# aymenboudhina/Multimodal_VQVAE_compression_audio_tactile

Hardware: AMD Instinct MI355X
Metric: encode+VQ+decode token-frames/sec (1 frame = 13.33 ms of paired 24 kHz audio+tactile) (higher is better)
Workload: dtype f32

## Files before the change

include/mvq.h:

```cpp
#ifndef MVQ_H
#define MVQ_H

#include <stddef.h>
#include <stdint.h>

#ifdef __cplusplus
extern "C" {
#endif

#define MVQ_OK 0
#define MVQ_EINVAL (-1)
#define MVQ_EUNSUPPORTED (-2)
#define MVQ_EHIP (-3)

#define MVQ_ACT_NONE 0
#define MVQ_ACT_TANH 1
#define MVQ_ACT_GELU 2

int mvq_abi_version(void);
const char* mvq_last_error(void);
unsigned mvq_build_flags(void);

typedef struct mvq_profile_entry {
    char kernel[96];
    double seconds;
    double flops;
    int launches;
} mvq_profile_entry;
int mvq_profile_begin(void);
int mvq_profile_end(mvq_profile_entry* out, int max_entries, int* n_entries);
int mvq_profile_end2(mvq_profile_entry* out, int max_entries, int* n_entries, int* n_total);
int mvq_profile_reserve(int n_launches);
int mvq_device_query(int* cu_count, int* lds_bytes_per_cu, char* arch, int arch_len);


int mvq_weight_norm_f32(const float* v, const float* g, float* w, int rows, int inner, void* stream);

size_t mvq_conv1d_packed_floats(int cin, int cout, int ks);
int mvq_conv1d_pack_f32(const float* w, float* wp, int cin, int cout, int ks, void* stream);

size_t mvq_conv_transpose1d_packed_floats(int cin, int cout, int stride);
int mvq_conv_transpose1d_pack_f32(const float* w, float* wp, int cin, int cout, int stride, void* stream);


int mvq_conv1d_f32(const float* x, const float* wp, const float* bias, const float* alpha_in,
                   const float* residual, const float* alpha_out, float* y,
                   int batch, int cin, int tin, int cout, int ks, int stride, int dil, int pad, int act,
                   void* stream);

int mvq_conv1d_dual_f32(const float* x, const float* wp, const float* bias, const float* alpha_in,
                        const float* residual, const float* alpha_out, float* y, float* y2, const float* alpha2,
                        int batch, int cin, int tin, int cout, int ks, int stride, int dil, int pad, int act,
                        void* stream);
int mvq_conv_transpose1d_dual_f32(const float* x, const float* wp, const float* bias, const float* alpha_in,
                                  const float* alpha_out, float* y, float* y2, const float* alpha2,
                                  int batch, int cin, int tin, int cout, int stride, int pad, void* stream);

int mvq_conv_kernel_name(int batch, int cin, int cout, int ks, int stride, int dil, int transposed, int tin,
                         char* buf, int len);

size_t mvq_residual_unit_scratch_floats(int batch, int c, int t, int dil);
int mvq_residual_unit_kernel_name(int c, int dil, char* buf, int len);
int mvq_residual_unit_f32(const float* x, const float* w7p, const float* b7, const float* alpha_a,
                          const float* alpha_b, const float* w1p, const float* b1, const float* alpha_next,
                          float* y, float* scratch, int batch, int c, int t, int dil, void* stream);

int mvq_residual_unit_dual_f32(const float* x, const float* x_snaked, const float* w7p, const float* b7,
                               const float* alpha_a, const float* alpha_b, const float* w1p, const float* b1,
                               const float* alpha_next, float* y, float* y2, const float* alpha2, float* scratch,
                               int batch, int c, int t, int dil, void* stream);

int mvq_conv_transpose1d_f32(const float* x, const float* wp, const float* bias, const float* alpha_in,
                             const float* alpha_out, float* y,
                             int batch, int cin, int tin, int cout, int stride, int pad, void* stream);


int mvq_rvq_ema_forward_f32(const float* z, const float* books, float* q_out, int32_t* idx_out,
                            int batch, int dim, int t, int nb_use, int k, void* stream);

size_t mvq_rvq_ema_step_scratch_bytes(int batch, int t, int nb, int k, int dim);
int mvq_rvq_ema_step_f32(const float* z_tokens, float* books, void* scratch,
                         int batch, int dim, int t, int nb, int k, float decay, void* stream);

int mvq_dac_rvq_f32(const float* z, const float* in_w, const float* in_b, const float* codebook,
                    const float* out_w, const float* out_b, float* zq, int32_t* codes, float* latents,
                    int batch, int c, int t, int nq_use, int k, int dc, void* stream);
int mvq_dac_rvq_items_f32(const float* z, const float* in_w, const float* in_b, const float* codebook,
                          const float* out_w, const float* out_b, float* zq, int32_t* codes, float* latents,
                          const int32_t* nq_item, int batch, int c, int t, int nq_use, int k, int dc, void* stream);
int mvq_dac_rvq_prepare_f32(const float* codebook, float* cb_normalised, float* cb_norm2, int nq, int k, int dc, void* stream);
int mvq_dac_rvq_prepared_f32(const float* z, const float* in_w, const float* in_b, const float* codebook,
                             const float* cb_normalised, const float* cb_norm2,
                             const float* out_w, const float* out_b, float* zq, int32_t* codes, float* latents,
                             const int32_t* nq_item, int batch, int c, int t, int nq_use, int k, int dc, void* stream);


int mvq_rvq_dequant_f32(const int64_t* idx, const float* books, float* q_out, int batch, int dim, int t, int nb_use, int k,
                        size_t out_sb, size_t out_sd, void* stream);
int mvq_dac_rvq_from_codes_f32(const int64_t* codes, const float* codebook, const float* out_w, const float* out_b, float* zq,
                               float* z_p, int batch, int c, int t, int nq_use, int k, int dc, void* stream);

int mvq_idx_pack_packets_u8(const int64_t* idx, uint8_t* bodies, int batch, int nb, int t, int k, int packet_tok,
                            size_t s_book, size_t s_item, void* stream);
int mvq_idx_unpack_packets(const uint8_t* bodies, const uint8_t* nb_recv, int64_t* idx, uint8_t* nb_valid, int batch, int nb, int t,
                           int k, int packet_tok, void* stream);
int mvq_rvq_dequant_layers_f32(const int64_t* idx, const float* books, const uint8_t* nb_valid, float* q_out, int batch, int dim,
                               int t, int nb_use, int k, size_t out_sb, size_t out_sd, void* stream);

#define MVQ_RATE_FULL 0
#define MVQ_RATE_TOL2 1
#define MVQ_RATE_BUDGET 2
int mvq_rvq_rate_f32(const float* z, size_t z_sb, size_t z_sd, const int32_t* idx, size_t idx_sbook, size_t idx_sitem,
// ... 257 lines not shown
```

multimodal_vqvae_compression_audio_tactile_amd/_lib.py:

```python
from __future__ import annotations

import ctypes
import subprocess
from ctypes import c_char_p, c_float, c_int, c_size_t, c_void_p
from pathlib import Path

_PKG = Path(__file__).resolve().parent
import os as _os
SO_PATH = Path(_os.environ["MVQ_LIB_PATH"]).resolve() if _os.environ.get("MVQ_LIB_PATH") else _PKG / "libmvq_hip.so"
_lib = None

class EncoderDesc(ctypes.Structure):
    _fields_ = [("d_model", c_int), ("n_strides", c_int), ("strides", c_int * 8), ("d_latent", c_int)]


class DecoderDesc(ctypes.Structure):
    _fields_ = [("input_channel", c_int), ("channels", c_int), ("n_rates", c_int), ("rates", c_int * 8), ("d_out", c_int), ("output_padding", c_int)]


class ArArgs(ctypes.Structure):
    _fields_ = ([(n, c_int) for n in ("batch", "t_lat", "t_audio", "tactile_only", "books_use", "rvq_k", "c_lat", "c_ff", "code_dim", "heads", "chunk")]
                + [(n, c_float) for n in ("ln_eps", "tok_eps", "scale")]
                + [(n, c_void_p) for n in ("zt", "k_all", "v_all", "pe", "lnq_g", "lnq_b", "wq", "wo", "lnf_g", "lnf_b", "w1", "b1", "w3", "b3",
                                           "tok_g", "tok_b", "wd", "bd", "wu", "bu", "books", "z_run", "r_tokens", "idx_out")])


class ProfileEntry(ctypes.Structure):
    _fields_ = [("kernel", ctypes.c_char * 96), ("seconds", ctypes.c_double), ("flops", ctypes.c_double), ("launches", c_int)]


EXPORTS = {
    "mvq_profile_begin": (c_int, []),
    "mvq_profile_end": (c_int, [ctypes.POINTER(ProfileEntry), c_int, ctypes.POINTER(c_int)]),
    "mvq_profile_end2": (c_int, [ctypes.POINTER(ProfileEntry), c_int, ctypes.POINTER(c_int), ctypes.POINTER(c_int)]),
    "mvq_profile_reserve": (c_int, [c_int]),
    "mvq_abi_version": (c_int, []),
    "mvq_build_flags": (ctypes.c_uint, []),
    "mvq_last_error": (c_char_p, []),
    "mvq_device_query": (c_int, [ctypes.POINTER(c_int), ctypes.POINTER(c_int), c_char_p, c_int]),
    "mvq_weight_norm_f32": (c_int, [c_void_p, c_void_p, c_void_p, c_int, c_int, c_void_p]),
    "mvq_conv1d_packed_floats": (c_size_t, [c_int, c_int, c_int]),
    "mvq_conv1d_pack_f32": (c_int, [c_void_p, c_void_p, c_int, c_int, c_int, c_void_p]),
    "mvq_conv_transpose1d_packed_floats": (c_size_t, [c_int, c_int, c_int]),
    "mvq_conv_transpose1d_pack_f32": (c_int, [c_void_p, c_void_p, c_int, c_int, c_int, c_void_p]),
    "mvq_conv_kernel_name": (c_int, [c_int] * 8 + [c_char_p, c_int]),
    "mvq_conv1d_f32": (c_int, [c_void_p] * 7 + [c_int] * 9 + [c_void_p]),
    "mvq_bf16x3_split_bytes": (c_size_t, [c_int] * 3),
    "mvq_bf16x3_split_f32": (c_int, [c_void_p, c_void_p, c_int, c_int, c_int, c_void_p]),
    "mvq_conv1d_k7_bf16x3_packed_bytes": (c_size_t, [c_int] * 2),
    "mvq_conv1d_k7_pack_bf16x3": (c_int, [c_void_p, c_void_p, c_int, c_int, c_int, c_void_p]),
    "mvq_conv1d_k7_bf16x6_f32": (c_int, [c_void_p] * 9 + [c_int] * 6 + [c_void_p]),
    "mvq_f16x2_split_f32": (c_int, [c_void_p, c_void_p, c_void_p, c_int, c_int, c_int, c_void_p]),
    "mvq_conv1d_k7_f16x2_packed_bytes": (c_size_t, [c_int] * 2),
    "mvq_conv1d_k7_pack_f16x2": (c_int, [c_void_p, c_void_p, c_void_p, c_int, c_int, c_int, c_void_p]),
    "mvq_conv1d_k7_f16x3_f32": (c_int, [c_void_p] * 11 + [c_int] * 6 + [c_void_p]),
    "mvq_residual_unit_scratch_floats": (c_size_t, [c_int] * 4),
    "mvq_residual_unit_kernel_name": (c_int, [c_int, c_int, c_char_p, c_int]),
    "mvq_residual_unit_f32": (c_int, [c_void_p] * 10 + [c_int] * 4 + [c_void_p]),
    "mvq_conv1d_dual_f32": (c_int, [c_void_p] * 9 + [c_int] * 9 + [c_void_p]),
    "mvq_conv_transpose1d_dual_f32": (c_int, [c_void_p] * 8 + [c_int] * 6 + [c_void_p]),
    "mvq_residual_unit_dual_f32": (c_int, [c_void_p] * 13 + [c_int] * 4 + [c_void_p]),
    "mvq_conv_transpose1d_f32": (c_int, [c_void_p] * 6 + [c_int] * 6 + [c_void_p]),
    "mvq_rvq_ema_forward_f32": (c_int, [c_void_p] * 4 + [c_int] * 5 + [c_void_p]),
    "mvq_rvq_ema_step_scratch_bytes": (c_size_t, [c_int] * 5),
    "mvq_rvq_ema_step_f32": (c_int, [c_void_p] * 3 + [c_int] * 5 + [c_float, c_void_p]),
    "mvq_dac_rvq_f32": (c_int, [c_void_p] * 9 + [c_int] * 6 + [c_void_p]),
    "mvq_dac_rvq_items_f32": (c_int, [c_void_p] * 10 + [c_int] * 6 + [c_void_p]),
    "mvq_dac_rvq_prepare_f32": (c_int, [c_void_p] * 3 + [c_int] * 3 + [c_void_p]),
    "mvq_dac_rvq_prepared_f32": (c_int, [c_void_p] * 12 + [c_int] * 6 + [c_void_p]),
    "mvq_rvq_dequant_f32": (c_int, [c_void_p] * 3 + [c_int] * 5 + [c_size_t] * 2 + [c_void_p]),
    "mvq_dac_rvq_from_codes_f32": (c_int, [c_void_p] * 6 + [c_int] * 6 + [c_void_p]),
    "mvq_idx_pack_packets_u8": (c_int, [c_void_p] * 2 + [c_int] * 5 + [c_size_t] * 2 + [c_void_p]),
    "mvq_idx_unpack_packets": (c_int, [c_void_p] * 4 + [c_int] * 5 + [c_void_p]),
    "mvq_fec_parity_u8": (c_int, [c_void_p] * 3 + [c_int] * 7 + [c_void_p]),
    "mvq_fec_recover_u8": (c_int, [c_void_p] * 5 + [c_int] * 7 + [c_void_p]),
    "mvq_fec_rs_parity_u8": (c_int, [c_void_p] * 3 + [c_int] * 8 + [c_void_p]),
    "mvq_fec_rs_recover_u8": (c_int, [c_void_p] * 5 + [c_int] * 8 + [c_void_p]),
    "mvq_rvq_dequant_layers_f32": (c_int, [c_void_p] * 4 + [c_int] * 5 + [c_size_t] * 2 + [c_void_p]),
    "mvq_rvq_rate_f32": (c_int, [c_void_p, c_size_t, c_size_t, c_void_p, c_size_t, c_size_t, c_void_p, c_void_p, c_size_t, c_size_t, c_void_p,
                                 c_size_t, c_void_p, c_size_t, c_void_p] + [c_int] * 9 + [c_float, c_int, c_void_p]),
    "mvq_dac_rvq_from_codes_layers_f32": (c_int, [c_void_p, c_size_t] + [c_void_p] * 6 + [c_int] * 6 + [c_void_p]),
    "mvq_dac_rvq_rate_workspace_bytes": (c_size_t, [c_int] * 4),
    "mvq_dac_rvq_rate_f32": (c_int, [c_void_p, c_void_p, c_size_t] + [c_void_p] * 8 + [c_size_t] + [c_int] * 9 + [c_float, c_int, c_void_p]),
    "mvq_layernorm_c_f32": (c_int, [c_void_p] * 5 + [c_int] * 3 + [c_size_t] * 2 + [c_float, c_int, c_float, c_void_p]),
    "mvq_attention_f32": (c_int, [c_void_p] * 4 + [c_int] * 5 + [c_size_t] * 4 + [c_void_p]),
    "mvq_align_xcorr_f32": (c_int, [c_void_p, c_void_p, c_int, c_int, c_void_p, c_void_p, c_void_p, c_void_p]),
    "mvq_align_xcorr_batch_f32": (c_int, [c_void_p, c_void_p, c_int, c_int, c_int, c_void_p, c_void_p, c_void_p, c_void_p]),
    "mvq_resample_ragged_f32": (c_int, [c_void_p] * 6 + [c_int] * 7 + [c_void_p]),
    "mvq_conv1d_dgrad_packed_floats": (c_size_t, [c_int] * 3),
    "mvq_conv1d_pack_dgrad_f32": (c_int, [c_void_p, c_void_p, c_int, c_int, c_int, c_void_p]),
    "mvq_conv_transpose1d_pack_dgrad_f32": (c_int, [c_void_p, c_void_p, c_int, c_int, c_int, c_void_p]),
    "mvq_conv1d_dgrad_f32": (c_int, [c_void_p] * 6 + [c_int] * 9 + [c_void_p]),
    "mvq_mul_dtanh_f32": (c_int, [c_void_p, c_void_p, c_void_p, c_size_t, c_void_p]),
    "mvq_layernorm_c_bwd_f32": (c_int, [c_void_p] * 8 + [c_int] * 3 + [c_size_t] * 2 + [c_float, c_void_p]),
    "mvq_gelu_bwd_f32": (c_int, [c_void_p, c_void_p, c_void_p, c_size_t, c_void_p]),
    "mvq_scale_tanh_f32": (c_int, [c_void_p, c_float, c_void_p, c_size_t, c_void_p]),
    "mvq_scale_tanh_bwd_f32": (c_int, [c_void_p, c_void_p, c_float, c_void_p, c_void_p, c_int, c_size_t, c_void_p]),
    "mvq_attention_bwd_f32": (c_int, [c_void_p] * 7 + [c_int] * 5 + [c_size_t] * 4 + [c_void_p]),
# ... 130 lines not shown
```

multimodal_vqvae_compression_audio_tactile_amd/csrc/api.hip:

```cpp
#include <hip/hip_runtime.h>
#include <stdarg.h>
#include <math.h>
#include <stdio.h>
#include <string.h>
#include "../../include/mvq.h"
#include "conv_dispatch.hpp"
#include "kernels_small.hpp"

#include <map>
#include <string>
#include <vector>

namespace mvq {
namespace {
struct ProfRec { std::string name; double flops; hipEvent_t e0, e1; };
std::vector<ProfRec> g_prof;
std::vector<hipEvent_t> g_prof_pool;
bool g_prof_on = false;
hipError_t g_prof_err = hipSuccess;
hipEvent_t prof_event()
{
    if (!g_prof_pool.empty()) { hipEvent_t e = g_prof_pool.back(); g_prof_pool.pop_back(); return e; }
    hipEvent_t e = nullptr;
    const hipError_t rc = hipEventCreate(&e);
// ... 260 lines not shown
size_t mvq_conv1d_k7_f16x2_packed_bytes(int cout, int cin)
{
    if (cout <= 0 || cin <= 0 || mvq::bf16x6_tile_rows(cout) == 0 || cin % 16 != 0) return 0;
    return (size_t)cout * cin * 7 * 4;
}
int mvq_conv1d_k7_pack_f16x2(const float* w, void* wq, uint32_t* wamax, int cout, int cin, int dgrad, void* stream)
{
    if (cout <= 0 || cin <= 0 || mvq::bf16x6_tile_rows(cout) == 0 || cin % 16 != 0)
        return fail(MVQ_EINVAL, "conv1d_k7_pack_f16x2: Cout %d must be a multiple of 128 or 96 and Cin %d of 16", cout, cin);
    if (!w || !wq || !wamax) return fail(MVQ_EINVAL, "conv1d_k7_pack_f16x2: null tensor");
    if ((reinterpret_cast<uintptr_t>(wq) & 15) != 0) return fail(MVQ_EINVAL, "conv1d_k7_pack_f16x2: wq must be 16-byte aligned");
    const hipError_t e = mvq::launch_f16x2_pack_k7(w, wq, wamax, cout, cin, dgrad != 0, S(stream));
    return e == hipSuccess ? MVQ_OK : hipfail(e, "conv1d_k7_pack_f16x2");
}
int mvq_conv1d_k7_f16x3_f32(const void* xs, const uint32_t* xamax, const void* wq, const uint32_t* wamax, const float* bias,
                            const float* alpha_out, float* y, float* y2, const float* dsn_src, const float* dsn_alpha,
                            const float* residual, int batch, int cin, int t, int cout, int dil, int tvalid, void* stream)
{
    if (batch < 0 || cin <= 0 || cout <= 0 || t < 0 || mvq::bf16x6_tile_rows(cout) == 0 || cin % 16 != 0)
        return fail(MVQ_EINVAL, "conv1d_k7_f16x3: bad shape B=%d Cin=%d T=%d Cout=%d (Cout %% 128 or 96, Cin %% 16)", batch, cin, t, cout);
    if (dil != 1 && dil != 3 && dil != 9) return fail(MVQ_EINVAL, "conv1d_k7_f16x3: dilation %d not in {1, 3, 9}", dil);
    if (tvalid < 0 || tvalid > t) return fail(MVQ_EINVAL, "conv1d_k7_f16x3: tvalid %d outside [0, %d]", tvalid, t);
    if (batch == 0 || t == 0) return MVQ_OK;
    if (!xs || !wq || !y || !xamax || !wamax) return fail(MVQ_EINVAL, "conv1d_k7_f16x3: null tensor");
    if (((reinterpret_cast<uintptr_t>(xs) | reinterpret_cast<uintptr_t>(wq)) & 15) != 0)
        return fail(MVQ_EINVAL, "conv1d_k7_f16x3: xs / wq must be 16-byte aligned");
    if ((long long)batch * ((t + 127) / 128) > 0x7fffffffLL) return fail(MVQ_EINVAL, "conv1d_k7_f16x3: grid too large");
    if (y2 && !alpha_out) return fail(MVQ_EINVAL, "conv1d_k7_f16x3: the dual output needs alpha_out");
    if ((dsn_src != nullptr) != (dsn_alpha != nullptr)) return fail(MVQ_EINVAL, "conv1d_k7_f16x3: dsn_src and dsn_alpha go together");
    mvq::K7Extra ex; ex.y2 = y2; ex.dsn_src = dsn_src; ex.dsn_alpha = dsn_alpha; ex.residual = residual;
    const hipError_t e = mvq::launch_conv_k7_f16x3(xs, xamax, wq, wamax, bias, alpha_out, y, batch, cin, t, cout, dil, tvalid, ex, S(stream));
    return e == hipSuccess ? MVQ_OK : hipfail(e, "conv1d_k7_f16x3");
}

int mvq_conv_kernel_name(int batch, int cin, int cout, int ks, int stride, int dil, int transposed, int tin, char* buf, int len)
{
    if (!buf || len <= 0) return fail(MVQ_EINVAL, "conv_kernel_name: bad buffer");
    mvq::ConvArgs a{};
    a.B = batch; a.Cin = cin; a.Tin = tin; a.Cout = cout; a.name_out = buf; a.name_len = len;
    hipError_t e;
    if (transposed) {
        a.Mrows = cout * stride; a.Mpad = mvq::conv_mpad(a.Mrows); a.Ncols = tin + 1; a.up_s = stride; a.pad = 1;
        e = dispatch_convtr(a, nullptr);
        if (e != hipSuccess) snprintf(buf, len, "convtr_direct_kernel");
    } else {
        const int pad = stride == 1 ? (ks - 1) * dil / 2 : (stride + 1) / 2;
        a.Mrows = cout; a.Mpad = mvq::conv_mpad(cout); a.Ncols = conv_out_len(tin, ks, stride, dil, pad); a.pad = pad;
        a.Tout = a.Ncols; a.up_s = 1;
        e = dispatch_conv1d(a, ks, stride, dil, nullptr);
        if (e != hipSuccess)
            snprintf(buf, len, "%s", (cin == 1 && ks == 7 && stride == 1 && dil == 1) ? "conv1d_cin1_kernel<7>"
                                   : (cout == 1 && ks == 7 && stride == 1 && dil == 1) ? "conv1d_cout1_kernel<7>"
                                                                                       : "conv1d_direct_kernel");
    }
    return MVQ_OK;
}

int mvq_conv1d_dual_f32(const float* x, const float* wp, const float* bias, const float* alpha_in,
                        const float* residual, const float* alpha_out, float* y, float* y2, const float* alpha2,
                        int batch, int cin, int tin, int cout, int ks, int stride, int dil, int pad, int act, void* stream);

int mvq_conv1d_f32(const float* x, const float* wp, const float* bias, const float* alpha_in,
                   const float* residual, const float* alpha_out, float* y,
                   int batch, int cin, int tin, int cout, int ks, int stride, int dil, int pad, int act, void* stream)
{
    return mvq_conv1d_dual_f32(x, wp, bias, alpha_in, residual, alpha_out, y, nullptr, nullptr,
                               batch, cin, tin, cout, ks, stride, dil, pad, act, stream);
}

int mvq_conv1d_dual_f32(const float* x, const float* wp, const float* bias, const float* alpha_in,
                        const float* residual, const float* alpha_out, float* y, float* y2, const float* alpha2,
                        int batch, int cin, int tin, int cout, int ks, int stride, int dil, int pad, int act, void* stream)
{
    return mvq_conv1d_padded_f32(x, wp, bias, alpha_in, residual, alpha_out, y, y2, alpha2, batch, cin, tin, cout, ks, stride,
                                 dil, pad, act, 0, stream);
}

int mvq_conv1d_padded_f32(const float* x, const float* wp, const float* bias, const float* alpha_in,
                          const float* residual, const float* alpha_out, float* y, float* y2, const float* alpha2,
                          int batch, int cin, int tin, int cout, int ks, int stride, int dil, int pad, int act, int tvalid,
                          void* stream)
{
    if (batch < 0 || cin <= 0 || cout <= 0 || tin < 0 || ks <= 0 || stride <= 0 || dil <= 0 || pad < 0)
        return fail(MVQ_EINVAL, "conv1d: bad shape B=%d Cin=%d Tin=%d Cout=%d ks=%d s=%d d=%d p=%d", batch, cin, tin, cout, ks, stride, dil, pad);
    if (act != MVQ_ACT_NONE && act != MVQ_ACT_TANH && act != MVQ_ACT_GELU) return fail(MVQ_EINVAL, "conv1d: bad act %d", act);
    const int tout = conv_out_len(tin, ks, stride, dil, pad);
    if (batch == 0 || tout == 0) return MVQ_OK;
    if (!x || !wp || !y) return fail(MVQ_EINVAL, "conv1d: null tensor");
    if ((y2 != nullptr) != (alpha2 != nullptr)) return fail(MVQ_EINVAL, "conv1d: y2 and alpha2 go together");
    if (tvalid < 0 || tvalid > tout) return fail(MVQ_EINVAL, "conv1d: tvalid %d outside [0, %d]", tvalid, tout);
    const int mpad = mvq::conv_mpad(cout);

    mvq::ConvArgs a{};
    a.x = x; a.wp = wp; a.bias = bias; a.alpha_in = alpha_in; a.residual = residual; a.alpha_out = alpha_out; a.y = y;
    a.B = batch; a.Cin = cin; a.Tin = tin; a.Cout = cout; a.Tout = tout; a.pad = pad; a.Mpad = mpad;
    a.Mrows = cout; a.Ncols = tout; a.act = act; a.up_s = 1; a.up_p = 0; a.y2 = y2; a.alpha2 = alpha2;
    a.tvalid = (tvalid == tout) ? 0 : tvalid;

    hipError_t e = dispatch_conv1d(a, ks, stride, dil, S(stream));
    if (e == hipErrorInvalidValue && (a.tvalid || act == MVQ_ACT_GELU))
        return fail(MVQ_EUNSUPPORTED, "conv1d: zero-padded rows / the GELU epilogue need an MFMA-tiled shape");
    if (e == hipErrorInvalidValue) {
        (void)hipGetLastError();
        mvq::DirectConvArgs d{x, wp, bias, alpha_in, residual, alpha_out, y, batch, cin, tin, cout, tout, ks, stride, dil, pad, mpad, act, y2, alpha2, nullptr, nullptr};
        e = mvq::launch_conv1d_direct(d, S(stream));
    }
// ... 1139 lines not shown
```

multimodal_vqvae_compression_audio_tactile_amd/csrc/conv_dispatch.hpp:

```cpp
#pragma once
#include "conv1d_mfma.hpp"

namespace mvq {
hipError_t launch_conv_k7(const ConvArgs& a, int dil, int bm, hipStream_t s);
hipError_t launch_conv_k1k3(const ConvArgs& a, int ks, int bm, hipStream_t s);
hipError_t launch_conv_strided(const ConvArgs& a, int stride, int bm, hipStream_t s);
hipError_t launch_conv_tr(const ConvArgs& a, int bm, hipStream_t s);
hipError_t launch_residual_unit_fused(const ConvArgs& a, int dil, hipStream_t s);
bool conv_lat_wanted(const ConvArgs& a, int ks);
hipError_t launch_conv_lat(const ConvArgs& a, int ks, int stride, int dil, hipStream_t s);
struct K7Extra {
    float* y2 = nullptr; const float* dsn_src = nullptr; const float* dsn_alpha = nullptr; const float* residual = nullptr;
};
hipError_t launch_bf16x3_split(const float* x, void* xs, int batch, int c, int t, hipStream_t s);
int bf16x6_tile_rows(int cout);
hipError_t launch_bf16x3_pack_k7(const float* w, void* wq, int cout, int cin, int flip, hipStream_t s);
hipError_t launch_conv_k7_bf16x6(const void* xs, const void* wq, const float* bias, const float* alpha_out, float* y, int batch, int cin,
                                 int t, int cout, int dil, int tvalid, const K7Extra& ex, hipStream_t s);
hipError_t launch_f16x2_split(const float* x, void* xs, unsigned* xamax, int batch, int c, int t, hipStream_t s);
hipError_t launch_f16x2_pack_k7(const float* w, void* wq, unsigned* wamax, int cout, int cin, int flip, hipStream_t s);
hipError_t launch_conv_k7_f16x3(const void* xs, const unsigned* xamax, const void* wq, const unsigned* wamax, const float* bias,
                                const float* alpha_out, float* y, int batch, int cin, int t, int cout, int dil, int tvalid, const K7Extra& ex,
                                hipStream_t s);
}
```

multimodal_vqvae_compression_audio_tactile_amd/csrc/conv_lat.hip:

```cpp
#include "conv_dispatch.hpp"
#include "conv_lat.hpp"

namespace mvq {

template <int KS, int STRIDE, int DIL, int CG>
__global__ __launch_bounds__(64) void conv1d_lat_kernel(const ConvArgs a)
{
    extern __shared__ __attribute__((aligned(16))) float lat_smem[];
    if (a.vec4) conv_lat_body<KS, STRIDE, DIL, CG, true>(a, blockIdx.x, blockIdx.y, lat_smem);
    else conv_lat_body<KS, STRIDE, DIL, CG, false>(a, blockIdx.x, blockIdx.y, lat_smem);
}

template <int KS, int STRIDE, int DIL, int CG>
static hipError_t launch_lat(const ConvArgs& a_in, hipStream_t s)
{
    using C = LatCfg<KS, STRIDE, DIL, CG>;
    ConvArgs a = a_in;
    if (a.Cin % CG != 0 || a.Mpad % 16 != 0) return hipErrorInvalidValue;
    if (a.name_out) {
        snprintf(a.name_out, a.name_len, "conv1d_lat_kernel<%d, %d, %d, %d>", KS, STRIDE, DIL, CG);
        return hipSuccess;
    }
    a.n_tiles = (a.Ncols + 15) / 16;
    a.vec4 = (a.Tin % 4 == 0) && ((reinterpret_cast<uintptr_t>(a.x) & 15) == 0);
    dim3 grid((unsigned)(a.n_tiles * a.B), (unsigned)((a.Mrows + 15) / 16));
    int pi = -1;
    if (prof_enabled()) {
        char nm[96];
        snprintf(nm, sizeof(nm), "conv1d_lat_kernel<%d, %d, %d, %d>", KS, STRIDE, DIL, CG);
        const int lim = a.tvalid > 0 ? a.tvalid : a.Ncols;
        pi = prof_begin(nm, 2.0 * a.Cin * KS * a.Mrows * (double)lim * a.B, s);
    }
    hipLaunchKernelGGL((conv1d_lat_kernel<KS, STRIDE, DIL, CG>), grid, dim3(64), (size_t)2 * C::BUF_FLOATS * sizeof(float), s, a);
    prof_end(pi, s);
    return hipGetLastError();
}

constexpr long LAT_MAX_TILES = 2048;

bool conv_lat_wanted(const ConvArgs& a, int ks)
{
    if (a.alpha_in || a.tper || a.vp_seg || a.up_per_out || a.n_base || a.n_tiles_max) return false;
    if (a.B <= 0 || a.Ncols <= 0 || a.up_s > 1) return false;
    const long tiles = (long)a.B * ((a.Ncols + 15) / 16) * ((a.Mrows + 15) / 16);
    const long steps = (long)a.Cin * ks / 4;
    if (tiles <= LAT_MAX_TILES / 2) return true;
    if (tiles <= LAT_MAX_TILES) return steps >= 512;
    return tiles <= 2 * LAT_MAX_TILES && steps >= 1536;
}

hipError_t launch_conv_lat(const ConvArgs& a, int ks, int stride, int dil, hipStream_t s)
{
    if (a.up_s > 1) return hipErrorInvalidValue;
    if (stride == 1) {
        if (ks == 1 && dil == 1) return a.Cin % 64 == 0 ? launch_lat<1, 1, 1, 64>(a, s) : launch_lat<1, 1, 1, 32>(a, s);
        if (ks == 3 && dil == 1) return launch_lat<3, 1, 1, 32>(a, s);
        if (ks == 7 && dil == 1) return launch_lat<7, 1, 1, 16>(a, s);
        if (ks == 7 && dil == 3) return launch_lat<7, 1, 3, 16>(a, s);
        if (ks == 7 && dil == 9) return launch_lat<7, 1, 9, 16>(a, s);
        return hipErrorInvalidValue;
    }
    if (dil != 1 || ks != 2 * stride) return hipErrorInvalidValue;
    switch (stride) {
        case 2: return launch_lat<4, 2, 1, 16>(a, s);
        case 4: return launch_lat<8, 4, 1, 8>(a, s);
        case 5: return launch_lat<10, 5, 1, 8>(a, s);
        case 8: return launch_lat<16, 8, 1, 8>(a, s);
    }
    return hipErrorInvalidValue;
}

}
```

multimodal_vqvae_compression_audio_tactile_amd/csrc/conv_lat.hpp:

```cpp
#pragma once
#include "conv1d_mfma.hpp"

namespace mvq {

template <int KS, int STRIDE, int DIL, int CG>
struct LatCfg {
    static constexpr int GS = CG * KS / 4;
    static constexpr int XT = 15 * STRIDE + (KS - 1) * DIL + 1;
    static constexpr int XV = (XT + 3 + 3) / 4;
    static constexpr int XTP = XV * 4 + 1;
    static constexpr int A_FLOATS = GS * 4 * 16;
    static constexpr int X_FLOATS = CG * XTP;
    static constexpr int BUF_FLOATS = (A_FLOATS + X_FLOATS + 3) / 4 * 4;
    static constexpr int A_V = A_FLOATS / 4;
    static constexpr int A_Q = (A_V + 63) / 64;
    static constexpr int X_Q = (CG * XV + 63) / 64;
    static constexpr int X_S = (CG * XT + 63) / 64;
    static_assert((CG * KS) % 4 == 0, "a group is a whole number of k-steps");
};

template <int KS, int STRIDE, int DIL, int CG, bool VEC, bool OPAQUE_TID = false>
__device__ __forceinline__ void conv_lat_body(const ConvArgs& a, int bx, int by, float* lat_smem)
{
    using C = LatCfg<KS, STRIDE, DIL, CG>;
    constexpr int GS = C::GS;
    int lane_ = threadIdx.x & 63;
    if (OPAQUE_TID) asm volatile("" : "+v"(lane_));
    const int lane = lane_;
    const int r = lane & 15, q = lane >> 4;
    const int b = bx / a.n_tiles, tn = bx - b * a.n_tiles;
    const int n0 = tn * 16, m0 = by * 16;
    const int n = n0 + r;
    const int t_in0 = n0 * STRIDE - a.pad;
    const int g_al = VEC ? (t_in0 & ~3) : t_in0;
    const int shift = t_in0 - g_al;
    const int ng = a.Cin / CG;

    constexpr int XN = VEC ? C::X_Q : C::X_S;
    constexpr int XTOT = VEC ? CG * C::XV : CG * C::XT;
    unsigned aoff[C::A_Q];
    unsigned xoff[XN], xlds[XN];
    unsigned xokm = 0;
#pragma unroll
    for (int u = 0; u < C::A_Q; ++u) {
        int e = lane + 64 * u;
        if (C::A_V % 64 != 0) e = e < C::A_V ? e : C::A_V - 1;
        aoff[u] = (unsigned)((e >> 2) * a.Mpad + 4 * (e & 3));
    }
#pragma unroll
    for (int u = 0; u < XN; ++u) {
        int e = lane + 64 * u;
        if (XTOT % 64 != 0) e = e < XTOT ? e : XTOT - 1;
        const int per = VEC ? C::XV : C::XT;
        const int cl = e / per, v = e - cl * per;
        const int t = g_al + (VEC ? 4 * v : v);
        const bool ok = t >= 0 && t < a.Tin;
        xoff[u] = (unsigned)(cl * a.Tin + (ok ? t : 0));
        xlds[u] = (unsigned)(C::A_FLOATS + cl * C::XTP + (VEC ? 4 * v : v));
        xokm |= ok ? (1u << u) : 0u;
    }
    static_assert(XN <= 32, "piece mask is 32 bits");
    const bool x_all_ok = __all(xokm == (XN == 32 ? 0xffffffffu : (1u << XN) - 1u));
    unsigned boff[GS];
#pragma unroll
    for (int p = 0; p < GS; ++p) {
        const int kl = 4 * p + q, cl = kl / KS, kk = kl - cl * KS;
        boff[p] = (unsigned)(C::A_FLOATS + cl * C::XTP + r * STRIDE + kk * DIL + shift);
    }

    const float* wsrc = a.wp + m0;
    const float* xsrc = a.x + (size_t)b * a.Cin * a.Tin;
    const size_t w_step = (size_t)(GS * 4) * a.Mpad, x_step = (size_t)CG * a.Tin;
    int g_next = 0;
    struct Stage { f32x4 w[C::A_Q]; f32x4 xq[VEC ? XN : 1]; float xs[VEC ? 1 : XN]; };
    auto gload = [&](Stage& S) __attribute__((always_inline)) {
#pragma unroll
        for (int u = 0; u < C::A_Q; ++u) S.w[u] = *reinterpret_cast<const f32x4*>(wsrc + aoff[u]);
#pragma unroll
        for (int u = 0; u < XN; ++u) {
            if constexpr (VEC) S.xq[u] = *reinterpret_cast<const f32x4*>(xsrc + xoff[u]);
            else S.xs[u] = xsrc[xoff[u]];
        }
        ++g_next;
        const bool more = g_next < ng;
        wsrc += more ? w_step : 0; xsrc += more ? x_step : 0;
    };
    auto lstore = [&](const Stage& S, float* buf) __attribute__((always_inline)) {
#pragma unroll
        for (int u = 0; u < C::A_Q; ++u)
            if (C::A_V % 64 == 0 || lane + 64 * u < C::A_V) *reinterpret_cast<f32x4*>(buf + (lane + 64 * u) * 4) = S.w[u];
#pragma unroll
        for (int u = 0; u < XN; ++u) {
            if (XTOT % 64 != 0 && lane + 64 * u >= XTOT) continue;
            const bool ok = x_all_ok || ((xokm >> u) & 1u);
            if constexpr (VEC) {
                float* d = buf + xlds[u];
                d[0] = ok ? S.xq[u].x : 0.0f; d[1] = ok ? S.xq[u].y : 0.0f; d[2] = ok ? S.xq[u].z : 0.0f; d[3] = ok ? S.xq[u].w : 0.0f;
            } else buf[xlds[u]] = ok ? S.xs[u] : 0.0f;
        }
    };
    struct Ops { float a[GS], b[GS]; };
    auto lread = [&](Ops& R, const float* buf) __attribute__((always_inline)) {
#pragma unroll
        for (int p = 0; p < GS; ++p) { R.a[p] = buf[p * 64 + lane]; R.b[p] = buf[boff[p]]; }
    };
    f32x4 acc = {0.0f, 0.0f, 0.0f, 0.0f};
    auto mfmas = [&](const Ops& R) __attribute__((always_inline)) {
#pragma unroll
        for (int p = 0; p < GS; ++p) acc = __builtin_amdgcn_mfma_f32_16x16x4f32(R.a[p], R.b[p], acc, 0, 0, 0);
    };
    constexpr int N_DSW = C::A_Q + (VEC ? 2 * XN : XN);
    constexpr int N_VM = C::A_Q + XN;
    auto interleave = [&]() __attribute__((always_inline)) {
#pragma unroll
        for (int p = 0; p < GS; ++p) {
            __builtin_amdgcn_sched_group_barrier(0x008, 1, 0);
            __builtin_amdgcn_sched_group_barrier(0x100, 2, 0);
            __builtin_amdgcn_sched_group_barrier(0x200, (N_DSW + GS - 1) / GS, 0);
            __builtin_amdgcn_sched_group_barrier(0x020, (N_VM + GS - 1) / GS, 0);
        }
    };
    float e_bias[4], e_res[4], e_dsn[4], e_dal[4], e_a2[4], e_al[4];
    bool e_ok[4];
#pragma unroll
    for (int i = 0; i < 4; ++i) {
        const int m = m0 + 4 * q + i;
        e_ok[i] = m < a.Mrows && n < a.Ncols;
        const int ch = e_ok[i] ? m : 0;
        const size_t off = e_ok[i] ? ((size_t)b * a.Cout + ch) * a.Tout + n : 0;
        e_bias[i] = a.bias ? a.bias[ch] : 0.0f;
        e_dsn[i] = a.dsn_src ? a.dsn_src[off] : 0.0f;
        e_dal[i] = a.dsn_src ? a.dsn_alpha[ch] : 0.0f;
        e_res[i] = a.residual ? a.residual[off] : 0.0f;
        e_a2[i] = a.y2 ? a.alpha2[ch] : 0.0f;
        e_al[i] = a.alpha_out ? a.alpha_out[ch] : 0.0f;
    }
    float* const buf0 = lat_smem;
    float* const buf1 = lat_smem + C::BUF_FLOATS;
    Stage S0, S1;
    Ops R0, R1;
    gload(S0);
    gload(S1);
    lstore(S0, buf0);
    gload(S0);
    __builtin_amdgcn_wave_barrier();
    lread(R0, buf0);
    lstore(S1, buf1);
    gload(S1);
    for (int g = 0; g < ng; g += 2) {
        __builtin_amdgcn_wave_barrier();
        lstore(S0, buf0);
        gload(S0);
        lread(R1, buf1);
        mfmas(R0);
        interleave();
        if (g + 1 < ng) {
            __builtin_amdgcn_wave_barrier();
            lstore(S1, buf1);
            gload(S1);
            lread(R0, buf0);
            mfmas(R1);
            interleave();
        }
    }

#pragma unroll
    for (int i = 0; i < 4; ++i) {
        if (!e_ok[i]) continue;
        const int ch = m0 + 4 * q + i, t = n;
        const size_t off = ((size_t)b * a.Cout + ch) * a.Tout + t;
        float v = acc[i] + e_bias[i];
        if (a.dsn_src) { const float ad = e_dal[i]; v = v * det_dsnake(e_dsn[i], ad, 1.0f / (ad + 1e-9f)); }
        if (a.residual) v = v + e_res[i];
        const bool tail = a.tvalid && t >= a.tvalid;
        if (a.y2) { const float a2 = e_a2[i]; a.y2[off] = tail ? 0.0f : det_snake(v, a2, 1.0f / (a2 + 1e-9f)); }
        if (a.alpha_out) { const float al = e_al[i]; v = det_snake(v, al, 1.0f / (al + 1e-9f)); }
        if (a.act == 1) v = det_tanh(v);
        if (a.act == 2) v = det_gelu(v);
        a.y[off] = tail ? 0.0f : v;
    }
}

}
```

multimodal_vqvae_compression_audio_tactile_amd/ops.py:

```python
from __future__ import annotations

import ctypes
import operator

import torch

from . import _lib
from ._lib import MvqError, check
from .stream import resample_stream_out_len


def _stream():
    return torch.cuda.current_stream().cuda_stream


def _dev(t: torch.Tensor, name: str) -> torch.Tensor:
    if not isinstance(t, torch.Tensor):
        raise TypeError(f"{name}: expected a torch.Tensor")
    if t.device.type != "cuda":
        raise MvqError(f"{name}: tensor is on {t.device}; the MI355X path has no CPU fallback")
    if t.dtype != torch.float32:
        t = t.float()
    return t.contiguous()


def _p(t):
    return None if t is None else t.data_ptr()


def conv1d_out_len(tin, ks, stride=1, dil=1, pad=0):
    span = tin + 2 * pad - dil * (ks - 1) - 1
    return 0 if span < 0 else span // stride + 1


def conv_kernel_name(cin, cout, ks, stride=1, dil=1, transposed=False, tin=24000, batch=64) -> str:
    import ctypes
    buf = ctypes.create_string_buffer(160)
    check(_lib.lib().mvq_conv_kernel_name(batch, cin, cout, ks, stride, dil, int(transposed), tin, buf, 160),
          "mvq_conv_kernel_name")
    return buf.value.decode()


def weight_norm(v: torch.Tensor, g: torch.Tensor) -> torch.Tensor:
    v = _dev(v, "v"); g = _dev(g, "g")
    w = torch.empty_like(v)
    rows = v.shape[0]
    check(_lib.lib().mvq_weight_norm_f32(v.data_ptr(), g.data_ptr(), w.data_ptr(), rows, v.numel() // rows, _stream()),
          "mvq_weight_norm_f32")
    return w


def pack_conv1d(w: torch.Tensor) -> torch.Tensor:
    w = _dev(w, "w")
    cout, cin, ks = w.shape
    n = _lib.lib().mvq_conv1d_packed_floats(cin, cout, ks)
    wp = torch.empty(n, device=w.device, dtype=torch.float32)
    check(_lib.lib().mvq_conv1d_pack_f32(w.data_ptr(), wp.data_ptr(), cin, cout, ks, _stream()), "mvq_conv1d_pack_f32")
    return wp


def pack_conv_transpose1d(w: torch.Tensor, stride: int) -> torch.Tensor:
    w = _dev(w, "w")
    cin, cout, ks = w.shape
    if ks != 2 * stride:
        raise MvqError(f"conv_transpose1d: kernel {ks} != 2*stride ({stride}) is outside the path")
    n = _lib.lib().mvq_conv_transpose1d_packed_floats(cin, cout, stride)
    wp = torch.empty(n, device=w.device, dtype=torch.float32)
    check(_lib.lib().mvq_conv_transpose1d_pack_f32(w.data_ptr(), wp.data_ptr(), cin, cout, stride, _stream()),
          "mvq_conv_transpose1d_pack_f32")
    return wp


def conv1d(x, wp, cout, ks, bias=None, stride=1, dil=1, pad=0, alpha_in=None, residual=None, alpha_out=None,
           tanh=False, out=None, alpha_dual=None, tvalid=0, gelu=False):
    x = _dev(x, "x")
    B, cin, tin = x.shape
    tout = conv1d_out_len(tin, ks, stride, dil, pad)
    if out is None:
        out = torch.empty(B, cout, tout, device=x.device, dtype=torch.float32)
    y2 = torch.empty_like(out) if alpha_dual is not None else None
    if residual is not None:
        residual = _dev(residual, "residual")
        if tuple(residual.shape) != (B, cout, tout):
            raise MvqError(f"conv1d: residual shape {tuple(residual.shape)} != {(B, cout, tout)}")
    check(_lib.lib().mvq_conv1d_padded_f32(x.data_ptr(), wp.data_ptr(), _p(bias), _p(alpha_in), _p(residual),
                                           _p(alpha_out), out.data_ptr(), _p(y2), _p(alpha_dual), B, cin, tin, cout, ks,
                                           stride, dil, pad, 1 if tanh else (2 if gelu else 0), int(tvalid), _stream()), "mvq_conv1d_f32")
    return out if alpha_dual is None else (out, y2)


def build_flags() -> int:
    return _lib.build_flags()

# ... 1697 lines not shown
```

Baseline: 61660.

## Share weight tiles across four waves in latent conv kernel via LDS

The latent conv kernel now uses a 4-wave workgroup for stride-1, ks>1 cases. The waves split the weight-slice loads between them and share the result through LDS, and each wave still owns its own input tile buffer. Block indices are remapped so groups of 8 row-tiles are laid out next to each other, and waves past the last tile only help load weights. This cuts redundant global weight traffic per wave, at the cost of block-wide __syncthreads instead of wave barriers, more LDS per block and more launch-geometry complexity. A plan query API is added for introspection.

```diff
diff --git a/include/mvq.h b/include/mvq.h
--- a/include/mvq.h
+++ b/include/mvq.h
@@ -58,6 +58,9 @@
 
 int mvq_conv_kernel_name(int batch, int cin, int cout, int ks, int stride, int dil, int transposed, int tin,
                          char* buf, int len);
+
+int mvq_conv_lat_plan(int batch, int cin, int cout, int ks, int stride, int dil, int tin, int* waves_per_group,
+                      int* grid_blocks);
 
 size_t mvq_residual_unit_scratch_floats(int batch, int c, int t, int dil);
 int mvq_residual_unit_kernel_name(int c, int dil, char* buf, int len);
diff --git a/multimodal_vqvae_compression_audio_tactile_amd/_lib.py b/multimodal_vqvae_compression_audio_tactile_amd/_lib.py
--- a/multimodal_vqvae_compression_audio_tactile_amd/_lib.py
+++ b/multimodal_vqvae_compression_audio_tactile_amd/_lib.py
@@ -44,6 +44,7 @@
     "mvq_conv_transpose1d_packed_floats": (c_size_t, [c_int, c_int, c_int]),
     "mvq_conv_transpose1d_pack_f32": (c_int, [c_void_p, c_void_p, c_int, c_int, c_int, c_void_p]),
     "mvq_conv_kernel_name": (c_int, [c_int] * 8 + [c_char_p, c_int]),
+    "mvq_conv_lat_plan": (c_int, [c_int] * 7 + [ctypes.POINTER(c_int)] * 2),
     "mvq_conv1d_f32": (c_int, [c_void_p] * 7 + [c_int] * 9 + [c_void_p]),
     "mvq_bf16x3_split_bytes": (c_size_t, [c_int] * 3),
     "mvq_bf16x3_split_f32": (c_int, [c_void_p, c_void_p, c_int, c_int, c_int, c_void_p]),
diff --git a/multimodal_vqvae_compression_audio_tactile_amd/csrc/api.hip b/multimodal_vqvae_compression_audio_tactile_amd/csrc/api.hip
--- a/multimodal_vqvae_compression_audio_tactile_amd/csrc/api.hip
+++ b/multimodal_vqvae_compression_audio_tactile_amd/csrc/api.hip
@@ -336,6 +336,24 @@
             snprintf(buf, len, "%s", (cin == 1 && ks == 7 && stride == 1 && dil == 1) ? "conv1d_cin1_kernel<7>"
                                    : (cout == 1 && ks == 7 && stride == 1 && dil == 1) ? "conv1d_cout1_kernel<7>"
                                                                                        : "conv1d_direct_kernel");
+    }
+    return MVQ_OK;
+}
+
+int mvq_conv_lat_plan(int batch, int cin, int cout, int ks, int stride, int dil, int tin, int* waves_per_group, int* grid_blocks)
+{
+    if (!waves_per_group || !grid_blocks) return fail(MVQ_EINVAL, "conv_lat_plan: null output");
+    *waves_per_group = 0; *grid_blocks = 0;
+    if (batch <= 0 || cin <= 0 || cout <= 0 || ks <= 0 || stride <= 0 || dil <= 0 || tin <= 0) return MVQ_OK;
+    mvq::ConvArgs a{};
+    const int pad = stride == 1 ? (ks - 1) * dil / 2 : (stride + 1) / 2;
+    a.B = batch; a.Cin = cin; a.Tin = tin; a.Cout = cout;
+    a.Mrows = cout; a.Mpad = mvq::conv_mpad(cout); a.Ncols = conv_out_len(tin, ks, stride, dil, pad); a.pad = pad;
+    a.Tout = a.Ncols; a.up_s = 1;
+    int nw = 0; long blocks = 0;
+    if (a.Cout >= 16 && a.Cin >= 32 && mvq::conv_underfilled(a) && mvq::conv_lat_wanted(a, ks) &&
+        mvq::conv_lat_plan(a, ks, stride, dil, &nw, &blocks) && blocks <= 0x7fffffffL) {
+        *waves_per_group = nw; *grid_blocks = (int)blocks;
     }
     return MVQ_OK;
 }
diff --git a/multimodal_vqvae_compression_audio_tactile_amd/csrc/conv_dispatch.hpp b/multimodal_vqvae_compression_audio_tactile_amd/csrc/conv_dispatch.hpp
--- a/multimodal_vqvae_compression_audio_tactile_amd/csrc/conv_dispatch.hpp
+++ b/multimodal_vqvae_compression_audio_tactile_amd/csrc/conv_dispatch.hpp
@@ -9,6 +9,7 @@
 hipError_t launch_residual_unit_fused(const ConvArgs& a, int dil, hipStream_t s);
 bool conv_lat_wanted(const ConvArgs& a, int ks);
 hipError_t launch_conv_lat(const ConvArgs& a, int ks, int stride, int dil, hipStream_t s);
+bool conv_lat_plan(const ConvArgs& a, int ks, int stride, int dil, int* waves_per_group, long* grid_blocks);
 struct K7Extra {
     float* y2 = nullptr; const float* dsn_src = nullptr; const float* dsn_alpha = nullptr; const float* residual = nullptr;
 };
diff --git a/multimodal_vqvae_compression_audio_tactile_amd/csrc/conv_lat.hip b/multimodal_vqvae_compression_audio_tactile_amd/csrc/conv_lat.hip
--- a/multimodal_vqvae_compression_audio_tactile_amd/csrc/conv_lat.hip
+++ b/multimodal_vqvae_compression_audio_tactile_amd/csrc/conv_lat.hip
@@ -3,27 +3,60 @@
 
 namespace mvq {
 
+constexpr int LAT_NW = 4;
+constexpr bool lat_has_shared(int ks, int stride) { return ks != 1 && stride == 1; }
+
 template <int KS, int STRIDE, int DIL, int CG>
-__global__ __launch_bounds__(64) void conv1d_lat_kernel(const ConvArgs a)
+__global__ __launch_bounds__(64 * LAT_NW) void conv1d_lat_kernel(const ConvArgs a)
 {
+    using C = LatCfg<KS, STRIDE, DIL, CG>;
     extern __shared__ __attribute__((aligned(16))) float lat_smem[];
-    if (a.vec4) conv_lat_body<KS, STRIDE, DIL, CG, true>(a, blockIdx.x, blockIdx.y, lat_smem);
-    else conv_lat_body<KS, STRIDE, DIL, CG, false>(a, blockIdx.x, blockIdx.y, lat_smem);
+    const int nw = (int)(blockDim.x >> 6);
+    const int gx = a.n_tiles * a.B;
+    const int gxg = (gx + nw - 1) / nw;
+    const int id = (int)blockIdx.x, j = id >> 3;
+    const int jy = lat_has_shared(KS, STRIDE) ? j / gxg : id / gxg;
+    const int by = lat_has_shared(KS, STRIDE) ? jy * 8 + (id & 7) : jy;
+    const int bxg = (lat_has_shared(KS, STRIDE) ? j : id) - jy * gxg;
+    if (by * 16 >= a.Mrows) return;
+    if (!lat_has_shared(KS, STRIDE) || nw == 1) {
+        if (a.vec4) conv_lat_body<KS, STRIDE, DIL, CG, true>(a, bxg, by, lat_smem);
+        else conv_lat_body<KS, STRIDE, DIL, CG, false>(a, bxg, by, lat_smem);
+    } else if constexpr (lat_has_shared(KS, STRIDE)) {
+        const int wv = __builtin_amdgcn_readfirstlane((int)(threadIdx.x >> 6));
+        float* const xs = lat_smem + 2 * C::wbuf_floats(LAT_NW) + wv * 2 * C::XBUF_FLOATS;
+        if (a.vec4) conv_lat_body<KS, STRIDE, DIL, CG, true, false, LAT_NW>(a, bxg * LAT_NW + wv, by, xs, lat_smem);
+        else conv_lat_body<KS, STRIDE, DIL, CG, false, false, LAT_NW>(a, bxg * LAT_NW + wv, by, xs, lat_smem);
+    }
 }
 
 template <int KS, int STRIDE, int DIL, int CG>
-static hipError_t launch_lat(const ConvArgs& a_in, hipStream_t s)
+static int lat_waves(const ConvArgs& a)
+{
+    (void)a;
+    return lat_has_shared(KS, STRIDE) ? LAT_NW : 1;
+}
+
+struct LatPlan { int waves = 0; long blocks = 0; };
+
+template <int KS, int STRIDE, int DIL, int CG>
+static hipError_t launch_lat(const ConvArgs& a_in, hipStream_t s, LatPlan* plan)
 {
     using C = LatCfg<KS, STRIDE, DIL, CG>;
+    static_assert(C::lds_bytes(LAT_NW) <= 64 * 1024 && C::lds_bytes(1) <= 64 * 1024, "dynamic LDS without an opt-in attribute");
     ConvArgs a = a_in;
     if (a.Cin % CG != 0 || a.Mpad % 16 != 0) return hipErrorInvalidValue;
+    a.n_tiles = (a.Ncols + 15) / 16;
+    const int nw = lat_waves<KS, STRIDE, DIL, CG>(a);
+    const long gx = (long)a.n_tiles * a.B, rt = (a.Mrows + 15) / 16;
+    const long blocks = 8 * ((rt + 7) / 8) * ((gx + nw - 1) / nw);
+    if (plan) { plan->waves = nw; plan->blocks = blocks; return hipSuccess; }
     if (a.name_out) {
         snprintf(a.name_out, a.name_len, "conv1d_lat_kernel<%d, %d, %d, %d>", KS, STRIDE, DIL, CG);
         return hipSuccess;
     }
-    a.n_tiles = (a.Ncols + 15) / 16;
+    if (blocks > 0x7fffffffL) return hipErrorInvalidValue;
     a.vec4 = (a.Tin % 4 == 0) && ((reinterpret_cast<uintptr_t>(a.x) & 15) == 0);
-    dim3 grid((unsigned)(a.n_tiles * a.B), (unsigned)((a.Mrows + 15) / 16));
     int pi = -1;
     if (prof_enabled()) {
         char nm[96];
@@ -31,7 +64,7 @@
         const int lim = a.tvalid > 0 ? a.tvalid : a.Ncols;
         pi = prof_begin(nm, 2.0 * a.Cin * KS * a.Mrows * (double)lim * a.B, s);
     }
-    hipLaunchKernelGGL((conv1d_lat_kernel<KS, STRIDE, DIL, CG>), grid, dim3(64), (size_t)2 * C::BUF_FLOATS * sizeof(float), s, a);
+    hipLaunchKernelGGL((conv1d_lat_kernel<KS, STRIDE, DIL, CG>), dim3((unsigned)blocks), dim3(64 * nw), C::lds_bytes(nw), s, a);
     prof_end(pi, s);
     return hipGetLastError();
 }
@@ -49,25 +82,38 @@
     return tiles <= 2 * LAT_MAX_TILES && steps >= 1536;
 }
 
-hipError_t launch_conv_lat(const ConvArgs& a, int ks, int stride, int dil, hipStream_t s)
+static hipError_t launch_conv_lat_impl(const ConvArgs& a, int ks, int stride, int dil, hipStream_t s, LatPlan* plan)
 {
     if (a.up_s > 1) return hipErrorInvalidValue;
     if (stride == 1) {
-        if (ks == 1 && dil == 1) return a.Cin % 64 == 0 ? launch_lat<1, 1, 1, 64>(a, s) : launch_lat<1, 1, 1, 32>(a, s);
-        if (ks == 3 && dil == 1) return launch_lat<3, 1, 1, 32>(a, s);
-        if (ks == 7 && dil == 1) return launch_lat<7, 1, 1, 16>(a, s);
-        if (ks == 7 && dil == 3) return launch_lat<7, 1, 3, 16>(a, s);
-        if (ks == 7 && dil == 9) return launch_lat<7, 1, 9, 16>(a, s);
+        if (ks == 1 && dil == 1) return a.Cin % 64 == 0 ? launch_lat<1, 1, 1, 64>(a, s, plan) : launch_lat<1, 1, 1, 32>(a, s, plan);
+        if (ks == 3 && dil == 1) return launch_lat<3, 1, 1, 32>(a, s, plan);
+        if (ks == 7 && dil == 1) return launch_lat<7, 1, 1, 16>(a, s, plan);
+        if (ks == 7 && dil == 3) return launch_lat<7, 1, 3, 16>(a, s, plan);
+        if (ks == 7 && dil == 9) return launch_lat<7, 1, 9, 16>(a, s, plan);
         return hipErrorInvalidValue;
     }
     if (dil != 1 || ks != 2 * stride) return hipErrorInvalidValue;
     switch (stride) {
-        case 2: return launch_lat<4, 2, 1, 16>(a, s);
-        case 4: return launch_lat<8, 4, 1, 8>(a, s);
-        case 5: return launch_lat<10, 5, 1, 8>(a, s);
-        case 8: return launch_lat<16, 8, 1, 8>(a, s);
+        case 2: return launch_lat<4, 2, 1, 16>(a, s, plan);
+        case 4: return launch_lat<8, 4, 1, 8>(a, s, plan);
+        case 5: return launch_lat<10, 5, 1, 8>(a, s, plan);
+        case 8: return launch_lat<16, 8, 1, 8>(a, s, plan);
     }
     return hipErrorInvalidValue;
 }
 
+hipError_t launch_conv_lat(const ConvArgs& a, int ks, int stride, int dil, hipStream_t s)
+{
+    return launch_conv_lat_impl(a, ks, stride, dil, s, nullptr);
 }
+
+bool conv_lat_plan(const ConvArgs& a, int ks, int stride, int dil, int* waves_per_group, long* grid_blocks)
+{
+    LatPlan p;
+    if (launch_conv_lat_impl(a, ks, stride, dil, nullptr, &p) != hipSuccess) return false;
+    *waves_per_group = p.waves; *grid_blocks = p.blocks;
+    return true;
+}
+
+}
diff --git a/multimodal_vqvae_compression_audio_tactile_amd/csrc/conv_lat.hpp b/multimodal_vqvae_compression_audio_tactile_amd/csrc/conv_lat.hpp
--- a/multimodal_vqvae_compression_audio_tactile_amd/csrc/conv_lat.hpp
+++ b/multimodal_vqvae_compression_audio_tactile_amd/csrc/conv_lat.hpp
@@ -17,36 +17,86 @@
     static constexpr int X_Q = (CG * XV + 63) / 64;
     static constexpr int X_S = (CG * XT + 63) / 64;
     static_assert((CG * KS) % 4 == 0, "a group is a whole number of k-steps");
+    static constexpr int A_CH = A_V / 64;
+    static constexpr int a_qw(int nw) { return (A_CH + nw - 1) / nw; }
+    static constexpr int wbuf_floats(int nw) { return a_qw(nw) * nw * 256; }
+    static constexpr int XBUF_FLOATS = (X_FLOATS + 3) / 4 * 4;
+    static constexpr size_t lds_bytes(int nw)
+    {
+        return sizeof(float) * (nw == 1 ? (size_t)2 * BUF_FLOATS : (size_t)2 * wbuf_floats(nw) + (size_t)nw * 2 * XBUF_FLOATS);
+    }
 };
 
-template <int KS, int STRIDE, int DIL, int CG, bool VEC, bool OPAQUE_TID = false>
-__device__ __forceinline__ void conv_lat_body(const ConvArgs& a, int bx, int by, float* lat_smem)
+template <int KS, int STRIDE, int DIL, int CG, bool VEC, bool OPAQUE_TID = false, int NW = 1>
+__device__ __forceinline__ void conv_lat_body(const ConvArgs& a, int bx, int by, float* lat_smem, float* w_smem = nullptr)
 {
     using C = LatCfg<KS, STRIDE, DIL, CG>;
     constexpr int GS = C::GS;
+    constexpr int AQ = NW == 1 ? C::A_Q : C::a_qw(NW);
+    constexpr int XB = NW == 1 ? C::A_FLOATS : 0;
+    static_assert(NW == 1 || C::A_V % 64 == 0, "the shared slice is dealt out in whole 64-piece chunks");
     int lane_ = threadIdx.x & 63;
     if (OPAQUE_TID) asm volatile("" : "+v"(lane_));
     const int lane = lane_;
     const int r = lane & 15, q = lane >> 4;
+    const int wv = NW == 1 ? 0 : __builtin_amdgcn_readfirstlane((int)(threadIdx.x >> 6));
+    const int ng = a.Cin / CG;
+    auto group_barrier = [&]() __attribute__((always_inline)) {
+        if constexpr (NW == 1) __builtin_amdgcn_wave_barrier(); else __syncthreads();
+    };
+    unsigned aoff[AQ];
+#pragma unroll
+    for (int u = 0; u < AQ; ++u) {
+        int e = lane + 64 * u;
+        if constexpr (NW == 1) { if (C::A_V % 64 != 0) e = e < C::A_V ? e : C::A_V - 1; }
+        else { const int c = wv + NW * u; e = lane + 64 * (c < C::A_CH ? c : C::A_CH - 1); }
+        aoff[u] = (unsigned)((e >> 2) * a.Mpad + 4 * (e & 3));
+    }
+    const unsigned wlds = (unsigned)(4 * lane + 256 * wv);
+    const float* wsrc = a.wp + by * 16;
+    const size_t w_step = (size_t)(GS * 4) * a.Mpad;
+    int g_next = 0;
+    if constexpr (NW > 1) {
+        if (bx >= a.n_tiles * a.B) {
+            f32x4 W0[AQ], W1[AQ];
+            auto wload = [&](f32x4* W) __attribute__((always_inline)) {
+#pragma unroll
+                for (int u = 0; u < AQ; ++u) W[u] = *reinterpret_cast<const f32x4*>(wsrc + aoff[u]);
+                ++g_next;
+                wsrc += g_next < ng ? w_step : 0;
+            };
+            auto wstore = [&](const f32x4* W, float* buf) __attribute__((always_inline)) {
+#pragma unroll
+                for (int u = 0; u < AQ; ++u) *reinterpret_cast<f32x4*>(buf + wlds + 256 * NW * u) = W[u];
+            };
+            float* const w0 = w_smem;
+            float* const w1 = w_smem + C::wbuf_floats(NW);
+            wload(W0); wload(W1);
+            wstore(W0, w0); wload(W0);
+            group_barrier();
+            wstore(W1, w1); wload(W1);
+            for (int g = 0; g < ng; g += 2) {
+                group_barrier();
+                wstore(W0, w0); wload(W0);
+                if (g + 1 < ng) {
+                    group_barrier();
+                    wstore(W1, w1); wload(W1);
+                }
+            }
+            return;
+        }
+    }
     const int b = bx / a.n_tiles, tn = bx - b * a.n_tiles;
     const int n0 = tn * 16, m0 = by * 16;
     const int n = n0 + r;
     const int t_in0 = n0 * STRIDE - a.pad;
     const int g_al = VEC ? (t_in0 & ~3) : t_in0;
     const int shift = t_in0 - g_al;
-    const int ng = a.Cin / CG;
 
     constexpr int XN = VEC ? C::X_Q : C::X_S;
     constexpr int XTOT = VEC ? CG * C::XV : CG * C::XT;
-    unsigned aoff[C::A_Q];
     unsigned xoff[XN], xlds[XN];
     unsigned xokm = 0;
-#pragma unroll
-    for (int u = 0; u < C::A_Q; ++u) {
-        int e = lane + 64 * u;
-        if (C::A_V % 64 != 0) e = e < C::A_V ? e : C::A_V - 1;
-        aoff[u] = (unsigned)((e >> 2) * a.Mpad + 4 * (e & 3));
-    }
 #pragma unroll
     for (int u = 0; u < XN; ++u) {
         int e = lane + 64 * u;
@@ -56,7 +106,7 @@
         const int t = g_al + (VEC ? 4 * v : v);
         const bool ok = t >= 0 && t < a.Tin;
         xoff[u] = (unsigned)(cl * a.Tin + (ok ? t : 0));
-        xlds[u] = (unsigned)(C::A_FLOATS + cl * C::XTP + (VEC ? 4 * v : v));
+        xlds[u] = (unsigned)(XB + cl * C::XTP + (VEC ? 4 * v : v));
         xokm |= ok ? (1u << u) : 0u;
     }
     static_assert(XN <= 32, "piece mask is 32 bits");
@@ -65,17 +115,15 @@
 #pragma unroll
     for (int p = 0; p < GS; ++p) {
         const int kl = 4 * p + q, cl = kl / KS, kk = kl - cl * KS;
-        boff[p] = (unsigned)(C::A_FLOATS + cl * C::XTP + r * STRIDE + kk * DIL + shift);
-    }
-
-    const float* wsrc = a.wp + m0;
+        boff[p] = (unsigned)(XB + cl * C::XTP + r * STRIDE + kk * DIL + shift);
+    }
+
     const float* xsrc = a.x + (size_t)b * a.Cin * a.Tin;
-    const size_t w_step = (size_t)(GS * 4) * a.Mpad, x_step = (size_t)CG * a.Tin;
-    int g_next = 0;
-    struct Stage { f32x4 w[C::A_Q]; f32x4 xq[VEC ? XN : 1]; float xs[VEC ? 1 : XN]; };
+    const size_t x_step = (size_t)CG * a.Tin;
+    struct Stage { f32x4 w[AQ]; f32x4 xq[VEC ? XN : 1]; float xs[VEC ? 1 : XN]; };
     auto gload = [&](Stage& S) __attribute__((always_inline)) {
 #pragma unroll
-        for (int u = 0; u < C::A_Q; ++u) S.w[u] = *reinterpret_cast<const f32x4*>(wsrc + aoff[u]);
+        for (int u = 0; u < AQ; ++u) S.w[u] = *reinterpret_cast<const f32x4*>(wsrc + aoff[u]);
 #pragma unroll
         for (int u = 0; u < XN; ++u) {
             if constexpr (VEC) S.xq[u] = *reinterpret_cast<const f32x4*>(xsrc + xoff[u]);
@@ -85,10 +133,12 @@
         const bool more = g_next < ng;
         wsrc += more ? w_step : 0; xsrc += more ? x_step : 0;
     };
-    auto lstore = [&](const Stage& S, float* buf) __attribute__((always_inline)) {
-#pragma unroll
-        for (int u = 0; u < C::A_Q; ++u)
-            if (C::A_V % 64 == 0 || lane + 64 * u < C::A_V) *reinterpret_cast<f32x4*>(buf + (lane + 64 * u) * 4) = S.w[u];
+    auto lstore = [&](const Stage& S, float* wbuf, float* buf) __attribute__((always_inline)) {
+#pragma unroll
+        for (int u = 0; u < AQ; ++u) {
+            if constexpr (NW == 1) { if (C::A_V % 64 == 0 || lane + 64 * u < C::A_V) *reinterpret_cast<f32x4*>(wbuf + (lane + 64 * u) * 4) = S.w[u]; }
+            else *reinterpret_cast<f32x4*>(wbuf + wlds + 256 * NW * u) = S.w[u];
+        }
 #pragma unroll
         for (int u = 0; u < XN; ++u) {
             if (XTOT % 64 != 0 && lane + 64 * u >= XTOT) continue;
@@ -100,17 +150,17 @@
         }
     };
     struct Ops { float a[GS], b[GS]; };
-    auto lread = [&](Ops& R, const float* buf) __attribute__((always_inline)) {
-#pragma unroll
-        for (int p = 0; p < GS; ++p) { R.a[p] = buf[p * 64 + lane]; R.b[p] = buf[boff[p]]; }
+    auto lread = [&](Ops& R, const float* wbuf, const float* buf) __attribute__((always_inline)) {
+#pragma unroll
+        for (int p = 0; p < GS; ++p) { R.a[p] = wbuf[p * 64 + lane]; R.b[p] = buf[boff[p]]; }
     };
     f32x4 acc = {0.0f, 0.0f, 0.0f, 0.0f};
     auto mfmas = [&](const Ops& R) __attribute__((always_inline)) {
 #pragma unroll
         for (int p = 0; p < GS; ++p) acc = __builtin_amdgcn_mfma_f32_16x16x4f32(R.a[p], R.b[p], acc, 0, 0, 0);
     };
-    constexpr int N_DSW = C::A_Q + (VEC ? 2 * XN : XN);
-    constexpr int N_VM = C::A_Q + XN;
+    constexpr int N_DSW = AQ + (VEC ? 2 * XN : XN);
+    constexpr int N_VM = AQ + XN;
     auto interleave = [&]() __attribute__((always_inline)) {
 #pragma unroll
         for (int p = 0; p < GS; ++p) {
@@ -136,29 +186,31 @@
         e_al[i] = a.alpha_out ? a.alpha_out[ch] : 0.0f;
     }
     float* const buf0 = lat_smem;
-    float* const buf1 = lat_smem + C::BUF_FLOATS;
+    float* const buf1 = lat_smem + (NW == 1 ? C::BUF_FLOATS : C::XBUF_FLOATS);
+    float* const w0 = NW == 1 ? buf0 : w_smem;
+    float* const w1 = NW == 1 ? buf1 : w_smem + C::wbuf_floats(NW);
     Stage S0, S1;
     Ops R0, R1;
     gload(S0);
     gload(S1);
-    lstore(S0, buf0);
+    lstore(S0, w0, buf0);
     gload(S0);
-    __builtin_amdgcn_wave_barrier();
-    lread(R0, buf0);
-    lstore(S1, buf1);
+    group_barrier();
+    lread(R0, w0, buf0);
+    lstore(S1, w1, buf1);
     gload(S1);
     for (int g = 0; g < ng; g += 2) {
-        __builtin_amdgcn_wave_barrier();
-        lstore(S0, buf0);
+        group_barrier();
+        lstore(S0, w0, buf0);
         gload(S0);
-        lread(R1, buf1);
+        lread(R1, w1, buf1);
         mfmas(R0);
         interleave();
         if (g + 1 < ng) {
-            __builtin_amdgcn_wave_barrier();
-            lstore(S1, buf1);
+            group_barrier();
+            lstore(S1, w1, buf1);
             gload(S1);
-            lread(R0, buf0);
+            lread(R0, w0, buf0);
             mfmas(R1);
             interleave();
         }
diff --git a/multimodal_vqvae_compression_audio_tactile_amd/ops.py b/multimodal_vqvae_compression_audio_tactile_amd/ops.py
--- a/multimodal_vqvae_compression_audio_tactile_amd/ops.py
+++ b/multimodal_vqvae_compression_audio_tactile_amd/ops.py
@@ -39,6 +39,16 @@
     check(_lib.lib().mvq_conv_kernel_name(batch, cin, cout, ks, stride, dil, int(transposed), tin, buf, 160),
           "mvq_conv_kernel_name")
     return buf.value.decode()
+
+
+def conv_lat_plan(cin, cout, ks, stride=1, dil=1, transposed=False, tin=24000, batch=64):
+    import ctypes
+    if transposed:
+        return 0, 0
+    nw, blocks = ctypes.c_int(0), ctypes.c_int(0)
+    check(_lib.lib().mvq_conv_lat_plan(batch, cin, cout, ks, stride, dil, tin, ctypes.byref(nw), ctypes.byref(blocks)),
+          "mvq_conv_lat_plan")
+    return nw.value, blocks.value
 
 
 def weight_norm(v: torch.Tensor, g: torch.Tensor) -> torch.Tensor:
```

Result: no change. 61650 (-0.0%).
